# swyoon/Diffusion-by-MaxEntIRL

Hardware: AMD Instinct MI355X
Metric: images/sec (CIFAR-10 DDPM T=10 generation) (higher is better)
Workload: dtype bf16; 1 GPU; CIFAR-10 DDPM U-Net (35.7M params) VARSampler T=10 generation, 256 images/GPU/step, 3x32x32 (BASELINE configs[1]); noise drawn inside the step; global_batch=256, T=10, parallelism=dp1 (independent trajectories, no collective)

## Files before the change

diffusion-by-maxentirl_amd/csrc/conv_ws8.hip:

```cpp
#include "conv_common.h"
#include <type_traits>


namespace {

constexpr int W8_HP = 10, W8_HS = 100;
constexpr int W8_HALO_BLOCKS = 25;
constexpr int W8_HALO = W8_HALO_BLOCKS * 1024;
constexpr int W8_A_SLOT = 4096;
#ifndef W8_RING_SLOTS
#define W8_RING_SLOTS 6
#endif
constexpr int W8_RING = W8_RING_SLOTS;
constexpr int W8_A_RING = W8_RING * W8_A_SLOT;
constexpr int W8_RO = 256 * 128;
constexpr int W8_TB = 2048;

__device__ uint4 w8_zero16 = {0u, 0u, 0u, 0u};

#define W8_GPTR(p) ((const __attribute__((address_space(1))) void*)(p))
#define W8_LPTR(p) ((__attribute__((address_space(3))) void*)(p))

__device__ __forceinline__ void w8_barrier() { asm volatile("s_waitcnt lgkmcnt(0)\n\ts_barrier" ::: "memory"); }

#define W8_INTERLEAVE_2()                                       \
    do {                                                        \
        _Pragma("unroll") for (int i_ = 0; i_ < 2; ++i_) {      \
            __builtin_amdgcn_sched_group_barrier(0x008, 3, 0);  \
            __builtin_amdgcn_sched_group_barrier(0x100, 1, 0);  \
        }                                                       \
        __builtin_amdgcn_sched_group_barrier(0x008, 2, 0);      \
    } while (0)
#define W8_INTERLEAVE_6()                                       \
    do {                                                        \
        _Pragma("unroll") for (int i_ = 0; i_ < 6; ++i_) {      \
            __builtin_amdgcn_sched_group_barrier(0x008, 1, 0);  \
            __builtin_amdgcn_sched_group_barrier(0x100, 1, 0);  \
        }                                                       \
        __builtin_amdgcn_sched_group_barrier(0x008, 2, 0);      \
    } while (0)

__device__ __forceinline__ void w8_wait_vm(int n) {
    switch (n >> 1) {
    case 0: asm volatile("s_waitcnt vmcnt(0)" ::: "memory"); break;
    case 1: asm volatile("s_waitcnt vmcnt(2)" ::: "memory"); break;
    case 2: asm volatile("s_waitcnt vmcnt(4)" ::: "memory"); break;
    case 3: asm volatile("s_waitcnt vmcnt(6)" ::: "memory"); break;
    case 4: asm volatile("s_waitcnt vmcnt(8)" ::: "memory"); break;
    case 5: asm volatile("s_waitcnt vmcnt(10)" ::: "memory"); break;
    default: asm volatile("s_waitcnt vmcnt(12)" ::: "memory"); break;
    }
}

struct W8Tile {
    int cot, n0;
};

template <bool GN>
__global__ __launch_bounds__(512, 1) void conv_ws8_kernel(ConvArgs p) {
    extern __shared__ __attribute__((aligned(1024))) char smem[];
    char* const halo0 = smem;
    char* const aring = smem + 2 * W8_HALO;
    char* const ro = aring + W8_A_RING;
    float* const tb = reinterpret_cast<float*>(ro + W8_RO);

    const int tid = threadIdx.x, lane = tid & 63;
    const int wave = __builtin_amdgcn_readfirstlane(tid >> 6);
    const int nchunks = (p.C0 + p.C1) / 32;
    const int S = 9 * nchunks;
    const int ntiles = p.PT * p.CT;

    auto tile_of = [&](int q, W8Tile& t) {
        t.cot = q % p.CT;
        t.n0 = (q / p.CT) * 4;
    };

    int q = dxmi_xcd_logical(blockIdx.x, gridDim.x, p.xcd_order);
    if (q >= ntiles) return;
    const int qstride = gridDim.x;

    if (wave < 4) {
        const int px = lane & 15, kg = lane >> 4;
        int bbase[3];
#pragma unroll
        for (int kx = 0; kx < 3; ++kx) {
            const int hx = (px & 7) + kx;
            bbase[kx] = ((wave * W8_HS + (px >> 3) * W8_HP + hx) * 64) + ((kg ^ (hx & 2)) << 4);
        }
        const char* const abase = aring + ((kg >> 1) * 2048) + ((px + 32 * (kg & 1)) << 4);
        f32x4 acc[4][4];
#pragma unroll
        for (int cb = 0; cb < 4; ++cb)
#pragma unroll
            for (int nb = 0; nb < 4; ++nb)
#pragma unroll
                for (int r = 0; r < 4; ++r) acc[cb][nb][r] = 0.f;
        bf16x8 A0[4], A1[4], Bx[2], By[2];
        auto read_a = [&](int u, bf16x8 (&A)[4]) {
            const char* as = abase + (u % W8_RING) * W8_A_SLOT;
#pragma unroll
            for (int cb = 0; cb < 4; ++cb) A[cb] = *reinterpret_cast<const bf16x8*>(as + (cb >> 1) * 1024 + (cb & 1) * 256);
        };
        auto read_b = [&](int u, int half, bf16x8 (&B)[2]) {
            const int t = u % 9, ky = t / 3, kx = t % 3;
            const char* hb = halo0 + ((u / 9) & 1) * W8_HALO + bbase[kx];
#pragma unroll
            for (int i = 0; i < 2; ++i) B[i] = *reinterpret_cast<const bf16x8*>(hb + ((2 * (half * 2 + i) + ky) * W8_HP) * 64);
        };
        auto mfma8 = [&](const bf16x8 (&A)[4], const bf16x8 (&B)[2], int half) {
#pragma unroll
            for (int i = 0; i < 2; ++i)
#pragma unroll
                for (int cb = 0; cb < 4; ++cb)
                    acc[cb][half * 2 + i] = __builtin_amdgcn_mfma_f32_16x16x32_bf16(A[cb], B[i], acc[cb][half * 2 + i], 0, 0, 0);
        };
        const float slope = dxmi_act_slope(p.act);
        const bool has_res = p.residual != nullptr;

        w8_barrier();
        read_a(0, A0);
        read_b(0, 0, Bx);
        for (;;) {
            const bool more = q + qstride < ntiles;
            f32x4 gam[4], bet[4];
            if constexpr (GN) {
                const int co0 = (q % p.CT) * 64 + 4 * kg;
#pragma unroll
                for (int cb = 0; cb < 4; ++cb) {
                    gam[cb] = *reinterpret_cast<const f32x4*>(p.gn_gamma + co0 + cb * 16);
                    bet[cb] = *reinterpret_cast<const f32x4*>(p.gn_beta + co0 + cb * 16);
                }
            }
            for (int c = 0; c < nchunks; c += 2) {
#pragma unroll
                for (int u = 0; u < 18; ++u) {
                    read_b(u, 1, By);
                    if (u & 1) mfma8(A1, Bx, 0); else mfma8(A0, Bx, 0);
                    W8_INTERLEAVE_2();
                    if (u % 3 == 2) w8_barrier();
                    if (u & 1) read_a(u + 1, A0); else read_a(u + 1, A1);
                    read_b(u + 1, 0, Bx);
                    if (u & 1) mfma8(A1, By, 1); else mfma8(A0, By, 1);
                    W8_INTERLEAVE_6();
                    __builtin_amdgcn_sched_barrier(0);
                }
            }
            w8_barrier();
            {
                const bool plain = p.act == DXMI_ACT_NONE;
                char* const rowb = ro + ((wave * 64 + px) << 7) + 8 * (kg & 1);
                auto epi = [&](auto RES, auto MASK, auto ACT) {
                    constexpr bool kRes = decltype(RES)::value, kMask = decltype(MASK)::value, kAct = decltype(ACT)::value;
#pragma unroll
                    for (int cb = 0; cb < 4; ++cb) {
                        const int co = cb * 16 + 4 * kg;
                        const f32x4 b0 = *reinterpret_cast<const f32x4*>(tb + co), t0 = *reinterpret_cast<const f32x4*>(tb + 64 + wave * 64 + co);
                        f32x4 bv;
#pragma unroll
                        for (int e = 0; e < 4; ++e) bv[e] = b0[e] + t0[e];
                        char* const a0 = rowb + (((cb * 2 + (kg >> 1)) ^ (px & 7)) << 4);
                        bf16x4 r[4];
                        if constexpr (kRes) {
#pragma unroll
                            for (int nb = 0; nb < 4; ++nb) r[nb] = *reinterpret_cast<const bf16x4*>(a0 + nb * 2048);
                        }
#pragma unroll
                        for (int nb = 0; nb < 4; ++nb) {
                            f32x4 v;
#pragma unroll
                            for (int e = 0; e < 4; ++e) v[e] = acc[cb][nb][e] + bv[e];
                            if constexpr (kRes) {
                                if constexpr (kMask) {
#pragma unroll
                                    for (int e = 0; e < 4; ++e) v[e] *= ((float)r[nb][e] > 0.f ? 1.f : p.mask_slope);
                                } else {
#pragma unroll
                                    for (int e = 0; e < 4; ++e) v[e] += (float)r[nb][e];
                                }
                            }
                            if constexpr (kAct) {
#pragma unroll
                                for (int e = 0; e < 4; ++e) v[e] = dxmi_act_lin(v[e], slope);
                            }
                            bf16x4 o;
#pragma unroll
                            for (int e = 0; e < 4; ++e) o[e] = (bf16)v[e];
                            if constexpr (GN) {
#pragma unroll
                                for (int e = 0; e < 4; ++e) acc[cb][nb][e] = (float)o[e];
                            } else {
                                *reinterpret_cast<bf16x4*>(a0 + nb * 2048) = o;
#pragma unroll
                                for (int e = 0; e < 4; ++e) acc[cb][nb][e] = 0.f;
                            }
                        }
                        if constexpr (GN) {
                            float s = 0.f;
#pragma unroll
                            for (int nb = 0; nb < 4; ++nb) s += (acc[cb][nb][0] + acc[cb][nb][1]) + (acc[cb][nb][2] + acc[cb][nb][3]);
                            s = dxmi_row16_sum(s);
                            s += __shfl_xor(s, 16, 64);
                            const float mean = s * (1.f / 512.f);
                            float qv = 0.f;
#pragma unroll
                            for (int nb = 0; nb < 4; ++nb) {
                                float d[4];
#pragma unroll
                                for (int e = 0; e < 4; ++e) d[e] = acc[cb][nb][e] - mean;
                                qv += (d[0] * d[0] + d[1] * d[1]) + (d[2] * d[2] + d[3] * d[3]);
                            }
                            qv = dxmi_row16_sum(qv);
                            qv += __shfl_xor(qv, 16, 64);
                            const float rstd = rsqrtf(qv * (1.f / 512.f) + p.gn_eps);
                            float ga[4], be[4];
#pragma unroll
                            for (int e = 0; e < 4; ++e) {
                                ga[e] = gam[cb][e] * rstd;
                                be[e] = bet[cb][e] - mean * ga[e];
                            }
#pragma unroll
                            for (int nb = 0; nb < 4; ++nb) {
                                bf16x4 y;
#pragma unroll
                                for (int e = 0; e < 4; ++e) {
                                    float t = acc[cb][nb][e] * ga[e] + be[e];
                                    if (p.gn_flags & 1) t = dxmi_silu_fast(t);
                                    y[e] = (bf16)t;
                                    acc[cb][nb][e] = 0.f;
                                }
                                *reinterpret_cast<bf16x4*>(a0 + nb * 2048) = y;
                            }
                        }
                    }
                };
                using T_ = std::true_type;
                using F_ = std::false_type;
                const bool is_mask = has_res && p.res_is_mask;
                if (plain && !is_mask) { if (has_res) epi(T_{}, F_{}, F_{}); else epi(F_{}, F_{}, F_{}); }
                else if (is_mask) { if (plain) epi(T_{}, T_{}, F_{}); else epi(T_{}, T_{}, T_{}); }
                else if (has_res) epi(T_{}, F_{}, T_{});
                else epi(F_{}, F_{}, T_{});
            }
            w8_barrier();
            if (!more) break;
            q += qstride;
        }
        return;
    }

    if (wave < 6) {
        const int lw = wave - 4;
        const char* const wb = reinterpret_cast<const char*>(p.w) + (size_t)lane * 16;
        W8Tile cur;
        tile_of(q, cur);
        auto issue_tap = [&](int cot, int g) {
            const int c = g / 9, t = g - c * 9;
            char* dst = aring + (g % W8_RING) * W8_A_SLOT + lw * 2048;
            const char* src = wb + ((size_t)(t * p.KST + c * 2 + lw) * p.CB + cot * 2) * 1024;
#pragma unroll
            for (int f = 0; f < 2; ++f)
                __builtin_amdgcn_global_load_lds(W8_GPTR(src + f * 1024), W8_LPTR(dst + f * 1024), 16, 0, 0);
        };
        static_assert(W8_RING == 6, "group hand-over needs the six-slot ring");
        u32x4 fq[2][3][2];
        auto load_tap = [&](int cot, int g, u32x4 (&f)[2]) {
            const int c = g / 9, t = g - c * 9;
            const char* src = wb + ((size_t)(t * p.KST + c * 2 + lw) * p.CB + cot * 2) * 1024;
#pragma unroll
            for (int k = 0; k < 2; ++k) asm volatile("global_load_dwordx4 %0, %1, off" : "=v"(f[k]) : "v"(src + k * 1024) : "memory");
        };
        auto store_tap = [&](int g, const u32x4 (&f)[2]) {
            char* dst = aring + (g % W8_RING) * W8_A_SLOT + lw * 2048 + lane * 16;
#pragma unroll
            for (int k = 0; k < 2; ++k) *reinterpret_cast<u32x4*>(dst + k * 1024) = f[k];
        };
        const int NG = S / 3;
        auto load_group = [&](int G, int cot_cur, int cot_nxt, u32x4 (&f)[3][2]) {
            const bool nx = G >= NG;
            const int g0 = (nx ? G - NG : G) * 3, cot = nx ? cot_nxt : cot_cur;
#pragma unroll
            for (int j = 0; j < 3; ++j) load_tap(cot, g0 + j, f[j]);
        };
        auto store_group = [&](int G, const u32x4 (&f)[3][2]) {
#pragma unroll
            for (int j = 0; j < 3; ++j) store_tap((G & 1) * 3 + j, f[j]);
        };
        const int t2l = lw * 64 + lane;
        const int kpc_l = (16 + nchunks - 2) / (nchunks - 1), pps_l = (kpc_l + 7) >> 3;
        const char* const zero_page_l = reinterpret_cast<const char*>(p.mask_src);
        auto piece_off_l = [&](const W8Tile& t, int k) -> long {
            const int lp = k * 16 + (t2l >> 3);
            const int c8 = (t2l & 7) ^ (lp & 7);
            const int n = t.n0 + (lp >> 6);
            if (n >= p.N) return -1;
            return (long)((((size_t)n * 8 + ((lp >> 3) & 7)) * 8 + (lp & 7)) * p.Cout + t.cot * 64 + c8 * 8);
        };
        bool first_tile_l = true;
        load_group(0, cur.cot, cur.cot, fq[0]);
        load_group(1, cur.cot, cur.cot, fq[1]);
        asm volatile("s_waitcnt vmcnt(6)" ::: "memory");
        store_group(0, fq[0]);
        asm volatile("s_waitcnt lgkmcnt(0)" ::: "memory");
        load_group(2, cur.cot, cur.cot, fq[0]);
        w8_barrier();
        for (;;) {
            const bool more = q + qstride < ntiles;
            W8Tile nxt = cur;
            if (more) tile_of(q + qstride, nxt);
            const bool res_here = !first_tile_l && p.residual != nullptr;
            first_tile_l = false;
            for (int G0 = 0; G0 < NG; G0 += 2) {
#pragma unroll
                for (int j = 0; j < 2; ++j) {
                    const int G = G0 + j;
                    asm volatile("s_waitcnt vmcnt(6)" ::: "memory");
                    store_group(G + 1, fq[(j + 1) & 1]);
                    asm volatile("s_waitcnt lgkmcnt(0)" ::: "memory");
                    if (res_here && G > 0) {
                        const int cg = (G - 1) / 3, g3 = (G - 1) - cg * 3;
                        if (cg + 1 < nchunks) {
                            const int k0 = cg * kpc_l < 16 ? cg * kpc_l : 16, k1 = k0 + kpc_l < 16 ? k0 + kpc_l : 16;
                            const int s0 = 3 * g3, s1 = g3 < 2 ? 3 * g3 + 3 : 8;
                            const int ka = k0 + s0 * pps_l < k1 ? k0 + s0 * pps_l : k1, kb = k0 + s1 * pps_l < k1 ? k0 + s1 * pps_l : k1;
#pragma unroll 1
                            for (int k = ka; k < kb; ++k) {
                                const long o = piece_off_l(cur, k);
                                const void* g = o >= 0 ? (const void*)(p.residual + o) : (const void*)zero_page_l;
                                __builtin_amdgcn_global_load_lds(W8_GPTR(g), W8_LPTR(ro + (k * 128 + lw * 64) * 16), 16, 0, 0);
                            }
                        }
                    }
                    load_group(G + 3, cur.cot, more ? nxt.cot : cur.cot, fq[(j + 1) & 1]);
                    w8_barrier();
                }
            }
            w8_barrier();
            w8_barrier();
            if (!more) break;
            q += qstride;
            cur = nxt;
        }
        asm volatile("s_waitcnt vmcnt(0)" ::: "memory");
        return;
    }

    {
        const int bw = wave - 6;
        const int t2 = bw * 64 + lane;
        constexpr int HB2 = (W8_HALO_BLOCKS + 1) / 2;
        const char* const zero_page = reinterpret_cast<const char*>(p.mask_src);
        int hoff0[HB2], hoff1[HB2];
        auto halo_plan = [&](const W8Tile& t) {
#pragma unroll
            for (int k = 0; k < HB2; ++k) {
                const int hp = (bw + 2 * k) * 16 + (lane >> 2);
                const int sub = hp / W8_HS, r = hp - sub * W8_HS;
                const int hy = r / W8_HP, hx = r - hy * W8_HP;
                const int iy = hy - 1, ix = hx - 1;
                const bool ok = sub < 4 && t.n0 + sub < p.N && iy >= 0 && ix >= 0 && iy < 8 && ix < 8;
                const int pix = p.ups ? ((t.n0 + sub) * 4 + (iy >> 1)) * 4 + (ix >> 1) : ((t.n0 + sub) * 8 + iy) * 8 + ix;
                const int j8 = ((lane & 3) ^ (hx & 2)) * 8;
                hoff0[k] = ok ? (pix * p.C0 + j8) * 2 : -1;
                hoff1[k] = ok ? (pix * p.C1 + j8) * 2 : -1;
            }
        };
        auto halo_issue = [&](int c, char* buf, int ka, int kb) {
            const int cbase = c * 32;
            const bool first = cbase < p.C0;
            const char* base = reinterpret_cast<const char*>(first ? p.in0 : p.in1) + (first ? cbase : cbase - p.C0) * 2;
#pragma unroll
            for (int k = 0; k < HB2; ++k) {
                if (k < ka || k >= kb) continue;
                const int blk = bw + 2 * k;
                const int off = first ? hoff0[k] : hoff1[k];
                const char* g = off >= 0 ? base + off : zero_page;
                if (blk < W8_HALO_BLOCKS)
                    __builtin_amdgcn_global_load_lds(W8_GPTR(g), W8_LPTR(buf + blk * 1024), 16, 0, 0);
            }
        };
        auto piece_off = [&](const W8Tile& t, int k) -> long {
            const int lp = k * 16 + (t2 >> 3);
            const int c8 = (t2 & 7) ^ (lp & 7);
            const int n = t.n0 + (lp >> 6);
            if (n >= p.N) return -1;
            return (long)((((size_t)n * 8 + ((lp >> 3) & 7)) * 8 + (lp & 7)) * p.Cout + t.cot * 64 + c8 * 8);
        };
        auto fetch_table = [&](const W8Tile& t) {
            if (bw != 0) return;
            if (p.bias) __builtin_amdgcn_global_load_lds(W8_GPTR(p.bias + t.cot * 64 + lane), W8_LPTR(tb), 4, 0, 0);
            if (p.addvec) {
#pragma unroll
                for (int sub = 0; sub < 4; ++sub) {
                    const int n = t.n0 + sub < p.N ? t.n0 + sub : p.N - 1;
                    __builtin_amdgcn_global_load_lds(W8_GPTR(p.addvec + (size_t)n * p.addvec_ld + t.cot * 64 + lane),
                                                     W8_LPTR(tb + 64 + sub * 64), 4, 0, 0);
                }
            }
        };
        bool do_res = p.residual != nullptr;
        auto fetch_residual = [&](const W8Tile& t, int k0, int k1) {
            if (!do_res) return;
#pragma unroll 1
            for (int k = k0; k < k1; ++k) {
                const long o = piece_off(t, k);
                const void* g = o >= 0 ? (const void*)(p.residual + o) : (const void*)zero_page;
                __builtin_amdgcn_global_load_lds(W8_GPTR(g), W8_LPTR(ro + (k * 128 + bw * 64) * 16), 16, 0, 0);
            }
        };
        auto tile_switch = [&](const W8Tile& pt, const W8Tile& ct, int k0, int k1) -> int {
#pragma unroll 1
            for (int k = k0; k < k1; k += 2) {
                const int n = k1 - k < 2 ? k1 - k : 2;
                bf16x8 v[2];
#pragma unroll
                for (int u = 0; u < 2; ++u)
                    if (u < n) v[u] = *reinterpret_cast<const bf16x8*>(ro + ((k + u) * 128 + t2) * 16);
#pragma unroll
                for (int u = 0; u < 2; ++u) {
                    const long o = u < n ? piece_off(pt, k + u) : -1;
                    if (u < n) {
                        if (o >= 0) *reinterpret_cast<bf16x8*>(reinterpret_cast<bf16*>(p.out) + o) = v[u];
                    }
                }
                fetch_residual(ct, k, k + n);
            }
            return (k1 - k0) * ((pt.n0 + 4 <= p.N ? 1 : 0) + (do_res ? 1 : 0));
        };

        W8Tile cur;
        tile_of(q, cur);
        if (bw == 0) {
            if (!p.bias) tb[lane] = 0.f;
            if (!p.addvec) { tb[64 + lane] = 0.f; tb[128 + lane] = 0.f; tb[192 + lane] = 0.f; tb[256 + lane] = 0.f; }
        }
        halo_plan(cur);
        halo_issue(0, halo0, 0, HB2);
        fetch_table(cur);
        fetch_residual(cur, 0, 16);
        if (do_res) asm volatile("s_waitcnt vmcnt(16)" ::: "memory");
        else asm volatile("s_waitcnt vmcnt(0)" ::: "memory");
        w8_barrier();
        do_res = false;
        bool have_prev = false;
        W8Tile prev = cur;
        const int kpc = (16 + nchunks - 2) / (nchunks - 1);
        const int pps = (kpc + 7) >> 3;
        for (;;) {
            const bool more = q + qstride < ntiles;
            W8Tile nxt = cur;
            if (more) tile_of(q + qstride, nxt);
            for (int c = 0; c < nchunks; ++c) {
                const bool wrap = c + 1 == nchunks;
                if (c == 0 && have_prev) fetch_table(cur);
                if (wrap && more) halo_plan(nxt);
                const bool do_halo = !wrap || more;
                char* const hbuf = halo0 + ((c + 1) & 1) * W8_HALO;
                const int hc = wrap ? 0 : c + 1;
                int k0 = 16, k1 = 16;
                if (have_prev && !wrap) {
                    k0 = c * kpc < 16 ? c * kpc : 16;
                    k1 = k0 + kpc < 16 ? k0 + kpc : 16;
                }
                int young = 0;
#pragma unroll
                for (int t = 0; t < 9; ++t) {
                    if (t < 7 && do_halo) halo_issue(hc, hbuf, 2 * t, 2 * t + 2);
                    if (t < 8) {
                        const int ka = k0 + t * pps < k1 ? k0 + t * pps : k1, kb = ka + pps < k1 ? ka + pps : k1;
                        if (ka < kb) {
                            const int n = tile_switch(prev, cur, ka, kb);
                            if (t >= 6) young += n;
                        }
                    }
                    if (t == 8) {
                        if (wrap) w8_wait_vm(0);
                        else w8_wait_vm(young);
                    }
                    if (t % 3 == 2) w8_barrier();
                }
            }
            w8_barrier();
            w8_barrier();
            prev = cur;
            have_prev = true;
            if (!more) break;
            q += qstride;
            cur = nxt;
        }
#pragma unroll 1
        for (int k = 0; k < 16; k += 4) {
            bf16x8 v[4];
#pragma unroll
            for (int u = 0; u < 4; ++u) v[u] = *reinterpret_cast<const bf16x8*>(ro + ((k + u) * 128 + t2) * 16);
#pragma unroll
            for (int u = 0; u < 4; ++u) {
                const long o = piece_off(prev, k + u);
                if (o >= 0) *reinterpret_cast<bf16x8*>(reinterpret_cast<bf16*>(p.out) + o) = v[u];
            }
        }
    }
}

}

bool conv_ws8_select(const ConvArgs& a, ConvPlan* p) {
    if (a.in_mode != DXMI_IN_NHWC_BF16 || a.out_mode != DXMI_OUT_NHWC_BF16) return false;
    if (a.ksize != 3 || a.stride != 1 || a.pad != 1 || a.ups == 2 || (a.mask_src && a.residual) || a.act == DXMI_ACT_SILU) return false;
    if (a.OH != 8 || a.OW != 8) return false;
    if (a.ups ? (a.IH != 4 || a.IW != 4) : (a.IH != 8 || a.IW != 8)) return false;
    if (a.Cout % 64 != 0 || (a.C0 + a.C1) % 32 != 0 || a.C0 % 32 != 0) return false;
    const int nchunks = (a.C0 + a.C1) / 32;
    if (nchunks < 4 || nchunks % 2 != 0 || (9 * nchunks) % W8_RING != 0) return false;
    if ((long)a.N * 64 * (a.C0 > a.C1 ? a.C0 : a.C1) * 2 >= (1L << 31)) return false;
    p->gn_out = (a.gn_flags & 2) != 0;
    if (a.gn_out && !p->gn_out) return false;
    ConvArgs& b = p->args;
    if (a.mask_src) { b.residual = a.mask_src; b.res_is_mask = 1; }
    if (a.gn_out) b.out = a.gn_out;
    b.SUBS = 4;
    b.PT = (a.N + 3) / 4;
    b.CT = a.Cout / 64;
    b.tile_px = 256;
    b.xcd_order = 1;
    p->kind = ConvKernel::ws8; p->t0 = a.gn_out != nullptr;
    p->grid = b.PT * b.CT < 256 ? b.PT * b.CT : 256;
    p->lds = 2 * W8_HALO + W8_A_RING + W8_RO + W8_TB;
    p->id = 400008;
    return true;
}

int conv_ws8_launch(const ConvPlan& p, hipStream_t st) {
    static const void* zero_page = nullptr;
    DXMI_CHECK_ARG(conv_zero_page(zero_page, HIP_SYMBOL(w8_zero16)), "dxmi_conv2d_fwd(ws8): hipGetSymbolAddress(w8_zero16) failed");
    ConvArgs b = p.args;
    b.mask_src = reinterpret_cast<const bf16*>(zero_page);
    static bool attr_set = false;
    if (!attr_set) {
        (void)hipFuncSetAttribute(reinterpret_cast<const void*>(conv_ws8_kernel<false>), hipFuncAttributeMaxDynamicSharedMemorySize, 160 * 1024);
        (void)hipFuncSetAttribute(reinterpret_cast<const void*>(conv_ws8_kernel<true>), hipFuncAttributeMaxDynamicSharedMemorySize, 160 * 1024);
        attr_set = true;
    }
    if (p.t0) hipLaunchKernelGGL(conv_ws8_kernel<true>, dim3(p.grid), dim3(512), p.lds, st, b);
    else hipLaunchKernelGGL(conv_ws8_kernel<false>, dim3(p.grid), dim3(512), p.lds, st, b);
    DXMI_CHECK_LAUNCH("dxmi_conv2d_fwd(ws8)");
    return DXMI_OK;
}
```

Before: 6632 images/s.

## Drop zero-padding border from ws8 halo; use pre-zeroed rows and shared zero strip

The LDS halo tile changes from a padded 10x10 layout to an unpadded 8-wide row layout. Top and bottom border rows are zeroed once at kernel start, and out-of-bounds columns point at a shared zero strip. Halo loads drop from 25 to 16 blocks per buffer, which cuts global_load_lds traffic for zero padding and removes the bounds logic. The cost is extra LDS for the strip and a one-time zeroing pass. Debug flags, compiled in only under DXMI_CONV_STAMPS, can skip loads or barriers for probing.

```diff
diff --git a/diffusion-by-maxentirl_amd/csrc/conv_ws8.hip b/diffusion-by-maxentirl_amd/csrc/conv_ws8.hip
--- a/diffusion-by-maxentirl_amd/csrc/conv_ws8.hip
+++ b/diffusion-by-maxentirl_amd/csrc/conv_ws8.hip
@@ -1,12 +1,15 @@
 #include "conv_common.h"
+#include <stdlib.h>
 #include <type_traits>
 
 
 namespace {
 
-constexpr int W8_HP = 10, W8_HS = 100;
-constexpr int W8_HALO_BLOCKS = 25;
-constexpr int W8_HALO = W8_HALO_BLOCKS * 1024;
+constexpr int W8_ROW = 8 * 64;
+constexpr int W8_IMG = 10 * W8_ROW;
+constexpr int W8_HALO_BLOCKS = 16;
+constexpr int W8_HALO = 4 * W8_IMG;
+constexpr int W8_STRIP = W8_IMG;
 constexpr int W8_A_SLOT = 4096;
 #ifndef W8_RING_SLOTS
 #define W8_RING_SLOTS 6
@@ -17,6 +20,12 @@
 constexpr int W8_TB = 2048;
 
 __device__ uint4 w8_zero16 = {0u, 0u, 0u, 0u};
+
+#ifdef DXMI_CONV_STAMPS
+#define W8_DBG(bit) (p.stagger & (bit))
+#else
+#define W8_DBG(bit) 0
+#endif
 
 #define W8_GPTR(p) ((const __attribute__((address_space(1))) void*)(p))
 #define W8_LPTR(p) ((__attribute__((address_space(3))) void*)(p))
@@ -60,7 +69,7 @@
 __global__ __launch_bounds__(512, 1) void conv_ws8_kernel(ConvArgs p) {
     extern __shared__ __attribute__((aligned(1024))) char smem[];
     char* const halo0 = smem;
-    char* const aring = smem + 2 * W8_HALO;
+    char* const aring = smem + 2 * W8_HALO + W8_STRIP;
     char* const ro = aring + W8_A_RING;
     float* const tb = reinterpret_cast<float*>(ro + W8_RO);
 
@@ -81,11 +90,15 @@
 
     if (wave < 4) {
         const int px = lane & 15, kg = lane >> 4;
-        int bbase[3];
+        int bbase[2][3];
 #pragma unroll
         for (int kx = 0; kx < 3; ++kx) {
-            const int hx = (px & 7) + kx;
-            bbase[kx] = ((wave * W8_HS + (px >> 3) * W8_HP + hx) * 64) + ((kg ^ (hx & 2)) << 4);
+            const int col = (px & 7) + kx - 1;
+            const int low = (px >> 3) * W8_ROW + ((kg ^ ((col & 4) >> 1)) << 4);
+            const bool inside = col >= 0 && col < 8;
+#pragma unroll
+            for (int b = 0; b < 2; ++b)
+                bbase[b][kx] = inside ? b * W8_HALO + wave * W8_IMG + col * 64 + low : 2 * W8_HALO + (col & 3) * 64 + low;
         }
         const char* const abase = aring + ((kg >> 1) * 2048) + ((px + 32 * (kg & 1)) << 4);
         f32x4 acc[4][4];
@@ -103,9 +116,9 @@
         };
         auto read_b = [&](int u, int half, bf16x8 (&B)[2]) {
             const int t = u % 9, ky = t / 3, kx = t % 3;
-            const char* hb = halo0 + ((u / 9) & 1) * W8_HALO + bbase[kx];
-#pragma unroll
-            for (int i = 0; i < 2; ++i) B[i] = *reinterpret_cast<const bf16x8*>(hb + ((2 * (half * 2 + i) + ky) * W8_HP) * 64);
+            const char* hb = halo0 + bbase[(u / 9) & 1][kx];
+#pragma unroll
+            for (int i = 0; i < 2; ++i) B[i] = *reinterpret_cast<const bf16x8*>(hb + (2 * (half * 2 + i) + ky) * W8_ROW);
         };
         auto mfma8 = [&](const bf16x8 (&A)[4], const bf16x8 (&B)[2], int half) {
 #pragma unroll
@@ -117,6 +130,13 @@
         const float slope = dxmi_act_slope(p.act);
         const bool has_res = p.residual != nullptr;
 
+        {
+            const uint4 z = {0u, 0u, 0u, 0u};
+#pragma unroll
+            for (int b = 0; b < 2; ++b)
+                *reinterpret_cast<uint4*>(halo0 + b * W8_HALO + wave * W8_IMG + (lane >> 5) * 9 * W8_ROW + (lane & 31) * 16) = z;
+            for (int i = wave; i < W8_STRIP / 1024; i += 4) *reinterpret_cast<uint4*>(halo0 + 2 * W8_HALO + i * 1024 + lane * 16) = z;
+        }
         w8_barrier();
         read_a(0, A0);
         read_b(0, 0, Bx);
@@ -137,7 +157,7 @@
                     read_b(u, 1, By);
                     if (u & 1) mfma8(A1, Bx, 0); else mfma8(A0, Bx, 0);
                     W8_INTERLEAVE_2();
-                    if (u % 3 == 2) w8_barrier();
+                    if (u % 3 == 2 && !(W8_DBG(4))) w8_barrier();
                     if (u & 1) read_a(u + 1, A0); else read_a(u + 1, A1);
                     read_b(u + 1, 0, Bx);
                     if (u & 1) mfma8(A1, By, 1); else mfma8(A0, By, 1);
@@ -264,6 +284,7 @@
         static_assert(W8_RING == 6, "group hand-over needs the six-slot ring");
         u32x4 fq[2][3][2];
         auto load_tap = [&](int cot, int g, u32x4 (&f)[2]) {
+            if (W8_DBG(1)) return;
             const int c = g / 9, t = g - c * 9;
             const char* src = wb + ((size_t)(t * p.KST + c * 2 + lw) * p.CB + cot * 2) * 1024;
 #pragma unroll
@@ -331,7 +352,7 @@
                         }
                     }
                     load_group(G + 3, cur.cot, more ? nxt.cot : cur.cot, fq[(j + 1) & 1]);
-                    w8_barrier();
+                    if (!(W8_DBG(4))) w8_barrier();
                 }
             }
             w8_barrier();
@@ -347,24 +368,23 @@
     {
         const int bw = wave - 6;
         const int t2 = bw * 64 + lane;
-        constexpr int HB2 = (W8_HALO_BLOCKS + 1) / 2;
+        constexpr int HB2 = W8_HALO_BLOCKS / 2;
         const char* const zero_page = reinterpret_cast<const char*>(p.mask_src);
         int hoff0[HB2], hoff1[HB2];
         auto halo_plan = [&](const W8Tile& t) {
 #pragma unroll
             for (int k = 0; k < HB2; ++k) {
-                const int hp = (bw + 2 * k) * 16 + (lane >> 2);
-                const int sub = hp / W8_HS, r = hp - sub * W8_HS;
-                const int hy = r / W8_HP, hx = r - hy * W8_HP;
-                const int iy = hy - 1, ix = hx - 1;
-                const bool ok = sub < 4 && t.n0 + sub < p.N && iy >= 0 && ix >= 0 && iy < 8 && ix < 8;
+                const int blk = bw + 2 * k;
+                const int sub = blk >> 2, iy = (blk & 3) * 2 + (lane >> 5), ix = (lane >> 2) & 7;
+                const bool ok = t.n0 + sub < p.N;
                 const int pix = p.ups ? ((t.n0 + sub) * 4 + (iy >> 1)) * 4 + (ix >> 1) : ((t.n0 + sub) * 8 + iy) * 8 + ix;
-                const int j8 = ((lane & 3) ^ (hx & 2)) * 8;
+                const int j8 = ((lane & 3) ^ ((ix & 4) >> 1)) * 8;
                 hoff0[k] = ok ? (pix * p.C0 + j8) * 2 : -1;
                 hoff1[k] = ok ? (pix * p.C1 + j8) * 2 : -1;
             }
         };
         auto halo_issue = [&](int c, char* buf, int ka, int kb) {
+            if (W8_DBG(2)) return;
             const int cbase = c * 32;
             const bool first = cbase < p.C0;
             const char* base = reinterpret_cast<const char*>(first ? p.in0 : p.in1) + (first ? cbase : cbase - p.C0) * 2;
@@ -374,8 +394,7 @@
                 const int blk = bw + 2 * k;
                 const int off = first ? hoff0[k] : hoff1[k];
                 const char* g = off >= 0 ? base + off : zero_page;
-                if (blk < W8_HALO_BLOCKS)
-                    __builtin_amdgcn_global_load_lds(W8_GPTR(g), W8_LPTR(buf + blk * 1024), 16, 0, 0);
+                __builtin_amdgcn_global_load_lds(W8_GPTR(g), W8_LPTR(buf + (blk >> 2) * W8_IMG + W8_ROW + (blk & 3) * 1024), 16, 0, 0);
             }
         };
         auto piece_off = [&](const W8Tile& t, int k) -> long {
@@ -464,19 +483,19 @@
                 int young = 0;
 #pragma unroll
                 for (int t = 0; t < 9; ++t) {
-                    if (t < 7 && do_halo) halo_issue(hc, hbuf, 2 * t, 2 * t + 2);
+                    if (t < 6 && do_halo) halo_issue(hc, hbuf, t < 2 ? 2 * t : t + 2, t < 2 ? 2 * t + 2 : t + 3);
                     if (t < 8) {
                         const int ka = k0 + t * pps < k1 ? k0 + t * pps : k1, kb = ka + pps < k1 ? ka + pps : k1;
                         if (ka < kb) {
                             const int n = tile_switch(prev, cur, ka, kb);
-                            if (t >= 6) young += n;
+                            if (t >= 5) young += n;
                         }
                     }
                     if (t == 8) {
                         if (wrap) w8_wait_vm(0);
                         else w8_wait_vm(young);
                     }
-                    if (t % 3 == 2) w8_barrier();
+                    if (t % 3 == 2 && !(W8_DBG(4))) w8_barrier();
                 }
             }
             w8_barrier();
@@ -524,7 +543,7 @@
     b.xcd_order = 1;
     p->kind = ConvKernel::ws8; p->t0 = a.gn_out != nullptr;
     p->grid = b.PT * b.CT < 256 ? b.PT * b.CT : 256;
-    p->lds = 2 * W8_HALO + W8_A_RING + W8_RO + W8_TB;
+    p->lds = 2 * W8_HALO + W8_STRIP + W8_A_RING + W8_RO + W8_TB;
     p->id = 400008;
     return true;
 }
@@ -534,6 +553,10 @@
     DXMI_CHECK_ARG(conv_zero_page(zero_page, HIP_SYMBOL(w8_zero16)), "dxmi_conv2d_fwd(ws8): hipGetSymbolAddress(w8_zero16) failed");
     ConvArgs b = p.args;
     b.mask_src = reinterpret_cast<const bf16*>(zero_page);
+#ifdef DXMI_CONV_STAMPS
+    static const int dbg = getenv("DXMI_CONV_WS8_DBG") ? atoi(getenv("DXMI_CONV_WS8_DBG")) : 0;
+    b.stagger = dbg;
+#endif
     static bool attr_set = false;
     if (!attr_set) {
         (void)hipFuncSetAttribute(reinterpret_cast<const void*>(conv_ws8_kernel<false>), hipFuncAttributeMaxDynamicSharedMemorySize, 160 * 1024);
```

After: 6721 images/s, median of 6. 1.01x the previous value.
